# UDC-GAC/pRIblast

Hardware: AMD Instinct MI355X
Metric: query RNAs/sec in `ris` step (higher is better)
Workload: dtype f64

## Files before the change

priblast_amd/csrc/gapped_lds.hip:

```cpp
#include <algorithm>
#include <type_traits>

#include "gapped_args.hpp"
#include "search_device.hpp"
#include "search_kernels.hpp"

namespace prb {

#ifdef PRB_GAP_PROFILE
constexpr int kProfSlots = 31;
__device__ unsigned long long g_gap_prof[10 * kProfSlots];
struct GapProf {
  unsigned long long last, acc[kProfSlots];
  int cells_now = 0, cells_prev = 0;
  __device__ __forceinline__ void start() {
    for (int i = 0; i < kProfSlots; i++) acc[i] = 0;
    last = __builtin_amdgcn_s_memtime();
  }
  __device__ __forceinline__ void mark(int r) {
    const unsigned long long t = __builtin_amdgcn_s_memtime();
    if (t >= last) acc[r] += t - last;
    else acc[29] += 1;
    last = t;
  }
  __device__ __forceinline__ void count(int r) { acc[r] += 1; }
  __device__ __forceinline__ void flush(int kind) {
    if ((threadIdx.x & 63) == 0)
      for (int i = 0; i < kProfSlots; i++) atomicAdd(&g_gap_prof[kind * kProfSlots + i], acc[i]);
  }
};
#define GP_MARK(r) prof.mark(r)
#define GP_COUNT(r) prof.count(r)
#else
struct GapProf {
  __device__ __forceinline__ void start() {}
  __device__ __forceinline__ void flush(int) {}
};
#define GP_MARK(r)
#define GP_COUNT(r)
#endif

namespace {

constexpr int kInitStage = 16;
struct Tier0 {
#ifndef PRB_T0_CAPR
#define PRB_T0_CAPR 48
#define PRB_T0_WGCU 4
#endif
#ifndef PRB_T0_ACC_GLOBAL
#define PRB_T0_ACC_GLOBAL false
#endif
  static constexpr int kG = 8, kCapD = 32, kCapR = PRB_T0_CAPR, kGroups = 32, kWavesPerSimd = PRB_T0_WGCU, kWgPerCu = PRB_T0_WGCU;
  static constexpr bool kResumable = true;
  static constexpr bool kResumes = false;
  static constexpr bool kPairSteps = true;
  static constexpr bool kAccGlobal = PRB_T0_ACC_GLOBAL;
};
#ifndef PRB_T12_ACC_GLOBAL
#define PRB_T12_ACC_GLOBAL true
#endif
#ifndef PRB_T12_WPS
#define PRB_T12_WPS (PRB_T12_ACC_GLOBAL ? 4 : 3)
#endif
#ifndef PRB_T1_CAPD
#define PRB_T1_CAPD 40
#define PRB_T1_CAPR 64
#define PRB_T1_GROUPS 32
#define PRB_T1_WGCU (PRB_T12_ACC_GLOBAL ? 4 : 3)
#endif
struct Tier1 {
  static constexpr int kG = 8, kCapD = PRB_T1_CAPD, kCapR = PRB_T1_CAPR, kGroups = PRB_T1_GROUPS, kWavesPerSimd = PRB_T12_WPS, kWgPerCu = PRB_T1_WGCU;
  static constexpr bool kResumable = true, kResumes = true;
  using From = Tier0;
  using FromRec = Rec32;
  static constexpr bool kPairSteps = false;
  static constexpr bool kAccGlobal = PRB_T12_ACC_GLOBAL;
};
struct Tier2 {
  static constexpr int kG = 16, kCapD = 64, kCapR = 120, kGroups = 16, kWavesPerSimd = PRB_T12_WPS, kWgPerCu = PRB_T12_ACC_GLOBAL ? 4 : 3;
  static constexpr bool kResumable = true, kResumes = true;
  using From = Tier1;
  using FromRec = Rec32;
  static constexpr bool kPairSteps = false;
  static constexpr bool kAccGlobal = PRB_T12_ACC_GLOBAL;
};
struct Tier3 {
  static constexpr int kG = 64, kCapD = 128, kCapR = 512, kGroups = 1, kWavesPerSimd = 4, kWgPerCu = 16;
  static constexpr bool kResumable = false, kResumes = true;
  using From = Tier2;
  using FromRec = Rec32;
  static constexpr bool kPairSteps = false;
  static constexpr bool kAccGlobal = false;
};

struct Rec32W {
  using word = uint32_t;
  static constexpr bool kBases = false;
  static __device__ __forceinline__ word pack(int i, int j, int pred, int type, int, int) {
    return (word)i | ((word)j << 8) | ((word)pred << 16) | ((word)type << 25);
  }
  static __device__ __forceinline__ int i(word v) { return v & 0xFF; }
  static __device__ __forceinline__ int j(word v) { return (v >> 8) & 0xFF; }
  static __device__ __forceinline__ int pred(word v) { return (v >> 16) & 0x1FF; }
  static __device__ __forceinline__ int type(word v) { return (v >> 25) & 7; }
  static __device__ __forceinline__ int qa(word) { return 0; }
  static __device__ __forceinline__ int da(word) { return 0; }
};
struct Rec64 {
  using word = uint64_t;
  static constexpr bool kBases = true;
  static __device__ __forceinline__ word pack(int i, int j, int pred, int type, int qa, int da) {
    return (word)(uint32_t)i | ((word)(uint32_t)j << 16) | ((word)type << 32) | ((word)qa << 36) | ((word)da << 40) |
           ((word)(uint32_t)pred << 44);
  }
  static __device__ __forceinline__ int i(word v) { return (int)(v & 0xFFFF); }
  static __device__ __forceinline__ int j(word v) { return (int)((v >> 16) & 0xFFFF); }
  static __device__ __forceinline__ int pred(word v) { return (int)(v >> 44); }
  static __device__ __forceinline__ int type(word v) { return (int)((v >> 32) & 0xF); }
  static __device__ __forceinline__ int qa(word v) { return (int)((v >> 36) & 0xF); }
  static __device__ __forceinline__ int da(word v) { return (int)((v >> 40) & 0xF); }
};
static_assert(Tier3::kCapD + 16 <= 255 && Tier3::kCapR <= 512 && Tier0::kCapR * 8 >= 6 * kInitStage * 4 && Tier2::kCapD + 16 <= 127 && Tier2::kCapR <= 127, "Rec32 field widths");
static_assert(Tier0::kCapD <= Tier1::kCapD && Tier1::kCapD <= Tier2::kCapD && Tier2::kCapD <= Tier3::kCapD && Tier0::kCapR <= Tier1::kCapR &&
                  Tier1::kCapR <= Tier2::kCapR && Tier2::kCapR <= Tier3::kCapR,
              "a tier continues the dumps of the one before it");

template <class T, class Rec> struct LdsState {
  double eq[T::kCapD], ed[T::kCapD];
  double hyb[T::kCapR];
  typename Rec::word info[T::kCapR];
  static constexpr int kPtabLen = (T::kCapD + 7) & ~7;
  alignas(8) uint8_t ptab[3][kPtabLen];
  uint8_t qb[T::kCapD + 16], db[T::kCapD + 16];
};
template <class T, class Rec, bool kAccGlobal = T::kAccGlobal> struct LdsLive : LdsState<T, Rec> {};
template <class T, class Rec> struct LdsLive<T, Rec, true> {
  double hyb[T::kCapR];
  typename Rec::word info[T::kCapR];
  static constexpr int kPtabLen = (T::kCapD + 7) & ~7;
  alignas(8) uint8_t ptab[3][kPtabLen];
  uint8_t qb[T::kCapD + 16], db[T::kCapD + 16];
};
template <class T, class Rec> struct LdsStore {
  using R = Rec;
  static constexpr bool kResumable = T::kResumable;
  static constexpr bool kAccGlobal = T::kAccGlobal;
  static constexpr int kCapD = T::kCapD, kCapR = T::kCapR;
  LdsLive<T, Rec> &s;
  double *acc;
  __device__ __forceinline__ int cap_d() const { return T::kCapD; }
  __device__ __forceinline__ int cap_r() const { return T::kCapR; }
  __device__ __forceinline__ double &eq(int i) const {
    if constexpr (T::kAccGlobal) return acc[i];
    else return s.eq[i];
  }
  __device__ __forceinline__ double &ed(int i) const {
    if constexpr (T::kAccGlobal) return acc[T::kCapD + i];
    else return s.ed[i];
  }
  __device__ __forceinline__ double &hyb(int r) const { return s.hyb[r]; }
  __device__ __forceinline__ typename Rec::word &info(int r) const { return s.info[r]; }
  __device__ __forceinline__ uint8_t &ptab(int row, int i) const { return s.ptab[row][i]; }
  __device__ __forceinline__ int ptab_len() const { return LdsState<T, Rec>::kPtabLen; }
  __device__ __forceinline__ int win_len() const { return T::kCapD + 16; }
  __device__ __forceinline__ uint8_t &qb(int t) const { return s.qb[t]; }
  __device__ __forceinline__ uint8_t &db(int t) const { return s.db[t]; }
};
struct HbmStore {
  using R = Rec64;
  static constexpr bool kResumable = false;
  static constexpr bool kAccGlobal = false;
  double *eq_, *ed_, *hyb_;
  uint64_t *info_;
  uint8_t *ptab_, *qb_, *db_;
  int capd, capr;
  __device__ __forceinline__ int cap_d() const { return capd; }
  __device__ __forceinline__ int cap_r() const { return capr; }
  __device__ __forceinline__ double &eq(int i) const { return eq_[i]; }
  __device__ __forceinline__ double &ed(int i) const { return ed_[i]; }
  __device__ __forceinline__ double &hyb(int r) const { return hyb_[r]; }
  __device__ __forceinline__ uint64_t &info(int r) const { return info_[r]; }
  __device__ __forceinline__ uint8_t &ptab(int row, int i) const { return ptab_[(size_t)row * (capd + 4) + i]; }
  __device__ __forceinline__ int ptab_len() const { return capd + 4; }
  __device__ __forceinline__ int win_len() const { return capd + 16; }
  __device__ __forceinline__ uint8_t &qb(int t) const { return qb_[t]; }
  __device__ __forceinline__ uint8_t &db(int t) const { return db_[t]; }
};

template <bool kLds> __device__ __forceinline__ void group_sync() {
  if (kLds) {
    __builtin_amdgcn_fence(__ATOMIC_RELEASE, "wavefront");
    __builtin_amdgcn_wave_barrier();
    __builtin_amdgcn_fence(__ATOMIC_ACQUIRE, "wavefront");
  } else {
    __builtin_amdgcn_fence(__ATOMIC_RELEASE, "workgroup");
    __builtin_amdgcn_wave_barrier();
    __builtin_amdgcn_fence(__ATOMIC_ACQUIRE, "workgroup");
  }
}

template <class Store> __device__ __forceinline__ void acc_sync() {
  if constexpr (Store::kAccGlobal) {
    __builtin_amdgcn_fence(__ATOMIC_RELEASE, "workgroup");
    __builtin_amdgcn_wave_barrier();
    __builtin_amdgcn_fence(__ATOMIC_ACQUIRE, "workgroup");
  }
}

template <int kCtrl> __device__ __forceinline__ double dpp_f64(double x) {
  const int lo = __builtin_amdgcn_update_dpp(0, __double2loint(x), kCtrl, 0xF, 0xF, false);
  const int hi = __builtin_amdgcn_update_dpp(0, __double2hiint(x), kCtrl, 0xF, 0xF, false);
  return __hiloint2double(hi, lo);
}
template <int kCtrl> __device__ __forceinline__ int dpp_i32(int x) { return __builtin_amdgcn_update_dpp(0, x, kCtrl, 0xF, 0xF, false); }
__device__ __forceinline__ void group_min_halves(double &te, int &key, bool halves) {
  double m = te;
  m = __builtin_fmin(m, dpp_f64<0xB1>(m));
  m = __builtin_fmin(m, dpp_f64<0x4E>(m));
  const double m8 = __builtin_fmin(m, dpp_f64<0x141>(m));
  m = halves ? m : m8;
  int k = te == m ? key : 0x7fffffff;
  k = min(k, dpp_i32<0xB1>(k));
  k = min(k, dpp_i32<0x4E>(k));
  const int k8 = min(k, dpp_i32<0x141>(k));
  te = m;
  key = halves ? k : k8;
}
template <int G> __device__ __forceinline__ void group_min(double &te, int &key) {
// ... 451 lines not shown
          if (te < bte) {
            bte = te;
            bkp = (k << 3) | R::type(v);
          }
        }
      }
    }
    GP_MARK(4);
    group_min<16>(bte, bkp);
    GP_MARK(5);
    int bk = bkp >> 3, ptype = bkp & 7;
    if (d.lo >= dstart) bk = 0;
    if (ptype == 0) ptype = R::type(S.info(bk));
    if (act && sl == 0) {
      const int rec = d.nrec + sub;
      S.hyb(rec) = bte;
      S.info(rec) = R::pack(ci, cj, bk, rtype_of(ctype), fq, fd);
      S.ptab(cur, ci) = (uint8_t)ptype;
    }
    const double ie = eq_c + ed_c + bte;
#pragma unroll
    for (int t = 0; t < 4; t++) {
      if (t < n) {
        const int l16 = 16 * t;
        const double ie_t = __hiloint2double(__builtin_amdgcn_readlane(__double2hiint(ie), l16), __builtin_amdgcn_readlane(__double2loint(ie), l16));
        const int ci_t = __builtin_amdgcn_readlane(ci, l16);
        if (ie_t < d.min_e) {
          d.min_e = ie_t;
          d.best = d.nrec + t;
          d.min_ci = ci_t;
          d.min_cj = d.length - ci_t;
        }
      }
    }
    d.nrec += n;
    GP_MARK(6);
  };

  auto cell_type = [&](int i) -> int {
    if (i > i_hi) return 0;
    const int j = d.length - i;
    const unsigned q0 = S.qb(i), d0 = S.db(j), q1 = S.qb(i + 1), d1 = S.db(j + 1), q2 = S.qb(i + 2), d2b = S.db(j + 2);
    const int pt = S.ptab(d2, i - 1);
    const unsigned x0 = q0 * 5 + d0, x1 = q1 * 5 + d1, x2 = q2 * 5 + d2b;
    const unsigned p0 = (sc.pair_mask >> x0) & 1, w0 = (sc.wobble_mask >> x0) & 1;
    unsigned ahead = 1;
    if (min_helix >= 2) ahead = ((sc.pair_mask >> x1) & 1) & ~(w0 & (sc.wobble_mask >> x1));
    if (min_helix >= 3) ahead &= sc.pair_mask >> x2;
    for (int x = 3; x <= min_helix - 1; x++) ahead &= sc.pair_mask >> ((unsigned)S.qb(i + x) * 5 + S.db(j + x));
    const unsigned need = (unsigned)(pt == 0) | (w0 & (unsigned)wobble(pt));
    int t = (int)((sc.bp_rows >> ((x0 * 3 - 15) & 63)) & 7);
    if (flag == 1) t = ((t - 1) ^ 1) + 1;
    return (p0 & (ahead | ~need) & 1) ? t : 0;
  };

  if constexpr (G == 8 && kLds) {
    constexpr int kChunks = (Store::kCapD + G - 1) / G;
    using cells_t = typename std::conditional<kChunks <= 4, uint32_t, unsigned long long>::type;
    uint32_t tw[kChunks];
    cells_t cells = 0;
#pragma unroll
    for (int c = 0; c < kChunks; c++) {
      tw[c] = 0;
      const int i0 = i_lo + c * G;
      if (i0 <= i_hi) {
        const int type1 = cell_type(i0 + gl);
        uint32_t w = (uint32_t)type1 << (3 * gl);
        w |= (uint32_t)dpp_i32<0xB1>((int)w);
        w |= (uint32_t)dpp_i32<0x4E>((int)w);
        w |= (uint32_t)dpp_i32<0x141>((int)w);
        tw[c] = w;
        cells |= (cells_t)((__ballot(type1 != 0) >> gbase) & 0xFF) << (8 * c);
        GP_COUNT(11);
      }
    }
    GP_MARK(3);
#ifdef PRB_GAP_PROFILE
    prof.cells_now = kChunks <= 4 ? __popc((uint32_t)cells) : __popcll((unsigned long long)cells);
#endif
    while (cells) {
      const cells_t rest = cells & (cells - 1);
      const bool two = rest != 0 && d.nrec + 2 <= S.cap_r();
      const int b0 = kChunks <= 4 ? __builtin_ctz((uint32_t)cells) : __builtin_ctzll((unsigned long long)cells);
      if (Store::kResumable && d.nrec >= S.cap_r()) {
        d.overflow = true;
        d.resume_i0 = i_lo + b0;
        d.resume_dstart = dstart;
        break;
      }
      int b = b0;
      if (two) {
        const int b1 = kChunks <= 4 ? __builtin_ctz((uint32_t)rest) : __builtin_ctzll((unsigned long long)rest);
        if (gl >= G / 2) b = b1;
        cells = rest & (rest - 1);
      } else {
        cells = rest;
      }
      uint32_t w = tw[0];
#pragma unroll
      for (int c = 1; c < kChunks; c++) w = (b >> 3) == c ? tw[c] : w;
      const int ptype = fill_cell(i_lo + b, (int)((w >> (3 * (b & 7))) & 7), two);
      if (ptype < 0) {
        d.overflow = true;
        break;
      }
    }
    group_sync<kLds>();
    GP_MARK(3);
  } else {
    for (int i0 = i_lo; i0 <= i_hi && !d.overflow; i0 += G) {
      const int type1 = cell_type(i0 + gl);
      using mask_t = typename std::conditional<G <= 32, uint32_t, unsigned long long>::type;
      const unsigned long long tb0 = __ballot(type1 & 1), tb1 = __ballot(type1 & 2), tb2 = __ballot(type1 & 4);
      const unsigned long long anyb = tb0 | tb1 | tb2;
      mask_t vmask = G < 64 ? (mask_t)((anyb >> gbase) & ((1ull << (G & 63)) - 1)) : (mask_t)anyb;
      GP_MARK(3);
      GP_COUNT(11);
      if (Store::kResumable && d.nrec + __popcll((unsigned long long)vmask) > S.cap_r()) {
        d.overflow = true;
        d.resume_i0 = i0;
        d.resume_dstart = dstart;
        break;
      }
      while (vmask) {
        if constexpr (G == 64) {
          const int left = __popcll((unsigned long long)vmask), n = left < 4 ? left : 4;
          if (n >= 2 && d.nrec + n <= S.cap_r()) {
            fill_quad(i0, (unsigned long long)vmask, n, tb0, tb1, tb2);
            for (int t = 0; t < n; t++) vmask &= vmask - 1;
            continue;
          }
        }
        const int b = G <= 32 ? __builtin_ctz((uint32_t)vmask) : __builtin_ctzll((unsigned long long)vmask);
        vmask &= vmask - 1;
        const int ctype = (int)((tb0 >> (gbase + b)) & 1) | (int)(((tb1 >> (gbase + b)) & 1) << 1) |
                          (int)(((tb2 >> (gbase + b)) & 1) << 2);
        const int ptype = fill_cell(i0 + b, ctype, false);
        if (ptype < 0) {
          d.overflow = true;
          break;
        }
      }
      group_sync<kLds>();
      GP_MARK(3);
    }
  }
  if (d.overflow) return true;
  if (d.length - (d.min_ci + d.min_cj) >= drop) return true;
  if (!q_open && !d_open) return true;
  return false;
}


struct PairStep {
  uint32_t cellsA, cellsB;
  int LA, loA, loB, dstartA, i_loA, curA, typeA0, nrec;
  bool paired;
};

__device__ __forceinline__ int nth_bit(uint32_t m, int r) {
  int pos = 0;
#pragma unroll
  for (int w = 16; w >= 1; w >>= 1) {
    const int c = __popc(m & ((1u << w) - 1));
    if (r >= c) {
      r -= c;
      m >>= w;
      pos += w;
    }
  }
  return pos;
}

template <class Store> __device__ __forceinline__ int pair_type(const SearchConst &sc, const Store &S, int flag, int i, int j) {
  const unsigned x0 = (unsigned)S.qb(i) * 5 + S.db(j);
  int t = (int)((sc.bp_rows >> ((x0 * 3 - 15) & 63)) & 7);
  if (flag == 1) t = ((t - 1) ^ 1) + 1;
  return t;
}

template <class Store>
__device__ __forceinline__ bool pair_prep(const SearchConst &sc, const SeqBases &sb, const ExtOpts &o, const HitCtx &c, int flag,
                                          const Store &S, int gl, int gbase, DirState &d, PairStep &p, GapProf &prof) {
  constexpr int G = 8;
  using R = typename Store::R;
  static_assert(Store::kCapD <= 32, "a 32-bit mask of cells per anti-diagonal");
  constexpr int kChunks = (Store::kCapD + G - 1) / G;
  const int delta = o.delta, drop = o.drop_w_gap, min_helix = o.min_helix;
  const bool mid = d.resume_i0 != 0;
  if (!mid) {
    if (d.length >= S.cap_d()) {
      d.overflow = true;
      return true;
    }
    d.length++;
  }
  const int LA = d.length;
  const bool openA = LA < d.tq0 || LA < d.td0;
  const int curA = LA - 3 * ((LA * 171) >> 9), d2A = curA == 2 ? 0 : curA + 1;
  if (!mid) {
    if (LA > d.staged) stage_acc_regs<G, true>(sb, c, flag, delta, S, gl, gbase, d, LA);
    GP_MARK(1);
    GP_COUNT(10);
    uint64_t *row = reinterpret_cast<uint64_t *>(&S.ptab(curA, 0));
    for (int t = gl; t < S.ptab_len() / 8; t += G) row[t] = 0;
    group_sync<true>();
    if (LA - 2 > drop) {
      while (d.lo < d.nrec) {
        const auto v = S.info(d.lo);
        if (LA - R::i(v) - R::j(v) - 2 > drop) d.lo++;
        else break;
      }
    }
  }
  GP_MARK(2);
  const int dstartA = mid ? d.resume_dstart : d.nrec, loA = d.lo;
  const int i_firstA = LA - d.td0 + 1 > 1 ? LA - d.td0 + 1 : 1;
  const int i_loA = mid ? d.resume_i0 : i_firstA;
  const int i_hiA = (LA < d.tq0 ? LA : d.tq0) - 1;
  d.resume_i0 = 0;

  auto helix_ok = [&](unsigned x0, unsigned x1, unsigned x2, int pt, int i, int j) -> bool {
    const unsigned p0 = (sc.pair_mask >> x0) & 1, w0 = (sc.wobble_mask >> x0) & 1;
    unsigned ahead = 1;
    if (min_helix >= 2) ahead = ((sc.pair_mask >> x1) & 1) & ~(w0 & (sc.wobble_mask >> x1));
    if (min_helix >= 3) ahead &= sc.pair_mask >> x2;
    for (int x = 3; x <= min_helix - 1; x++) ahead &= sc.pair_mask >> ((unsigned)S.qb(i + x) * 5 + S.db(j + x));
    const unsigned need = (unsigned)(pt == 0) | (w0 & (unsigned)wobble(pt));
    return (p0 & (ahead | ~need) & 1) != 0;
  };

  const int LB = LA + 1, d2B = curA == 0 ? 2 : curA - 1;
  const bool try_pair = !mid && openA && LA - (d.min_ci + d.min_cj) < drop && LA < S.cap_d() && LB <= d.staged;
  uint32_t cellsA = 0, cellsB = 0;
  int loB = loA;
  bool paired = false;
  if (try_pair) {
    if (LB - 2 > drop) {
      while (loB < dstartA) {
        const auto v = S.info(loB);
        if (LB - R::i(v) - R::j(v) - 2 > drop) loB++;
        else break;
      }
    }
    const int i_loB = LB - d.td0 + 1 > 1 ? LB - d.td0 + 1 : 1, i_hiB = (LB < d.tq0 ? LB : d.tq0) - 1;
#pragma unroll
    for (int ch = 0; ch < kChunks; ch++) {
      const int i0 = i_loA + ch * G;
      if (i0 <= i_hiB) {
        const int i = i0 + gl, j = LA - i, jc = j < 0 ? 0 : j;
        const unsigned q0 = (unsigned)S.qb(i) * 5, q1 = (unsigned)S.qb(i + 1) * 5, q2 = (unsigned)S.qb(i + 2) * 5;
        const unsigned d0 = S.db(jc), d1 = S.db(jc + 1), d2b = S.db(jc + 2), d3 = S.db(jc + 3);
        const bool okA = i <= i_hiA && helix_ok(q0 + d0, q1 + d1, q2 + d2b, S.ptab(d2A, i - 1), i, j);
        const bool okB = i >= i_loB && i <= i_hiB && helix_ok(q0 + d1, q1 + d2b, q2 + d3, S.ptab(d2B, i - 1), i, j + 1);
        cellsA |= (uint32_t)((__ballot(okA) >> gbase) & 0xFF) << (8 * ch);
        cellsB |= (uint32_t)((__ballot(okB) >> gbase) & 0xFF) << (8 * ch);
        GP_COUNT(11);
      }
    }
    if (d.nrec + __popc(cellsA) + __popc(cellsB) <= S.cap_r()) {
      paired = true;
      uint64_t *row = reinterpret_cast<uint64_t *>(&S.ptab(d2A, 0));
      for (int t = gl; t < S.ptab_len() / 8; t += G) row[t] = 0;
      group_sync<true>();
      GP_COUNT(10);
    } else {
      cellsB = 0;
    }
  } else {
#pragma unroll
    for (int ch = 0; ch < kChunks; ch++) {
      const int i0 = i_loA + ch * G;
      if (i0 <= i_hiA) {
        const int i = i0 + gl, j = LA - i, jc = j < 0 ? 0 : j;
        const unsigned x0 = (unsigned)S.qb(i) * 5 + S.db(jc), x1 = (unsigned)S.qb(i + 1) * 5 + S.db(jc + 1),
                       x2 = (unsigned)S.qb(i + 2) * 5 + S.db(jc + 2);
        const bool okA = i <= i_hiA && helix_ok(x0, x1, x2, S.ptab(d2A, i - 1), i, j);
        cellsA |= (uint32_t)((__ballot(okA) >> gbase) & 0xFF) << (8 * ch);
        GP_COUNT(11);
      }
    }
  }
  const int nA = __popc(cellsA);
  int typeA0 = 0;
  if (paired && nA != 0) {
    const int iA0 = i_loA + __builtin_ctz(cellsA);
    typeA0 = rtype_of(pair_type(sc, S, flag, iA0, LA - iA0));
  }
#ifdef PRB_GAP_PROFILE
  prof.cells_now = nA + __popc(cellsB);
#endif
  const int room = S.cap_r() - d.nrec;
  if (nA > room) {
    const int keep = room > 0 ? room : 0, b = nth_bit(cellsA, keep);
    cellsA &= (1u << b) - 1;
    d.overflow = true;
    if (Store::kResumable) {
      d.resume_i0 = i_loA + b;
      d.resume_dstart = dstartA;
    }
  }
  p.cellsA = cellsA;
  p.cellsB = cellsB;
  p.LA = LA;
  p.loA = loA;
  p.loB = loB;
  p.dstartA = dstartA;
  p.i_loA = i_loA;
  p.curA = curA;
  p.typeA0 = typeA0;
  p.nrec = d.nrec;
  p.paired = paired;
  GP_MARK(3);
  return false;
}

template <class Store>
__device__ __forceinline__ void pair_cell(const SearchConst &sc, const Store &S, int flag, const PairStep &p, int b, int rec, int sub,
                                          int stride, bool halves, bool act, GapProf &prof) {
  using R = typename Store::R;
  GP_COUNT(12);
  const bool isB = b >= 32;
  const int cur = isB ? (p.curA == 2 ? 0 : p.curA + 1) : p.curA;
  const int lo = act ? (isB ? p.loB : p.loA) : 0, dstart = act ? p.dstartA : 0;
  const int ci = act ? p.i_loA + (b & 31) : 1, cj = act ? p.LA + (isB ? 1 : 0) - ci : 1;
  const int ctype = pair_type(sc, S, flag, ci, cj);
  const int nq = S.qb(ci - 1), nd = S.db(cj - 1);
  double bte = 1000000.0;
  int bkp = lo << 3;
  const typename R::word v0 = lo + sub < dstart ? S.info(lo + sub) : 0;
  scan_qualifying<R>(
      S, lo, dstart, sub, stride, ci, cj, v0,
      [&](typename R::word v) -> double {
        const int ri = R::i(v), rj = R::j(v);
        const int rq = R::qa(v), rd = R::da(v);
        const bool f0 = flag == 0;
        const int rt = R::type(v);
        return loop_energy_abcd(sc, f0 ? ctype : rt, f0 ? rt : ctype, ci - ri - 1, cj - rj - 1, f0 ? nq : rq, f0 ? nd : rd,
                                f0 ? rq : nq, f0 ? rd : nd);
      },
      bte, bkp, prof);
  GP_MARK(4);
  group_min_halves(bte, bkp, halves);
  GP_MARK(5);
  int bk = bkp >> 3, ptype = bkp & 7;
  const bool a_first = isB && p.typeA0 != 0 && lo >= dstart;
  if (lo >= dstart && !a_first) bk = 0;
  if (ptype == 0) ptype = a_first ? p.typeA0 : R::type(S.info(bk));
  if (act && sub == 0) {
    S.hyb(rec) = bte;
    S.info(rec) = R::pack(ci, cj, bk, rtype_of(ctype), S.qb(ci + 1), S.db(cj + 1));
    S.ptab(cur, ci) = (uint8_t)ptype;
  }
  GP_MARK(6);
}

template <class Store>
__device__ __forceinline__ void pair_fill_group(const SearchConst &sc, const Store &S, int flag, const PairStep &p, int gl, GapProf &prof) {
  unsigned long long cells = (unsigned long long)p.cellsA | ((unsigned long long)p.cellsB << 32);
  int rec = p.nrec;
  while (cells) {
    const unsigned long long rest = cells & (cells - 1);
    const bool two = rest != 0, hi = two && gl >= 4;
    const int b = hi ? __builtin_ctzll(rest) : __builtin_ctzll(cells);
    pair_cell(sc, S, flag, p, b, rec + (hi ? 1 : 0), two ? (gl & 3) : gl, two ? 4 : 8, two, true, prof);
    cells = two ? rest & (rest - 1) : rest;
    rec += two ? 2 : 1;
  }
  GP_MARK(26);
  group_sync<true>();
}

template <class T, class Rec>
__device__ __forceinline__ void pair_fill_pool(const SearchConst &sc, LdsLive<T, Rec> *wave_lds, int flag, const PairStep &p, int lane,
                                               GapProf &prof) {
  static_assert(T::kG == 8 && !T::kAccGlobal && T::kCapD < 255 && T::kCapR < 256, "eight groups per wavefront, state in LDS, 8-bit fields");
  const int n = __popc(p.cellsA) + __popc(p.cellsB);
  int incl[8];
  int total = 0;
#pragma unroll
  for (int g = 0; g < 8; g++) {
    total += __builtin_amdgcn_readlane(n, 8 * g);
    incl[g] = total;
  }
  group_sync<true>();
  const uint32_t pk0 = (uint32_t)p.LA | ((uint32_t)p.loA << 8) | ((uint32_t)p.loB << 16) | ((uint32_t)p.dstartA << 24);
  const uint32_t pk1 = (uint32_t)p.i_loA | ((uint32_t)p.curA << 8) | ((uint32_t)p.typeA0 << 10) | ((uint32_t)flag << 13) | ((uint32_t)p.nrec << 16);
  const int slot = lane >> 2, sub = lane & 3;
  for (int t0 = 0; t0 < total; t0 += 16) {
    GP_COUNT(30);
    const int t = t0 + slot;
    int o = 0, ex = 0;
#pragma unroll
    for (int g = 0; g < 7; g++) {
      if (t >= incl[g]) {
        o = g + 1;
        ex = incl[g];
      }
    }
    const int ob = 8 * o;
    const uint32_t q0 = __shfl(pk0, ob), q1 = __shfl(pk1, ob), cA = __shfl(p.cellsA, ob), cB = __shfl(p.cellsB, ob);
    PairStep po;
    po.cellsA = cA;
    po.cellsB = cB;
    po.LA = q0 & 0xFF;
    po.loA = (q0 >> 8) & 0xFF;
    po.loB = (q0 >> 16) & 0xFF;
    po.dstartA = q0 >> 24;
    po.i_loA = q1 & 0xFF;
    po.curA = (q1 >> 8) & 3;
    po.typeA0 = (q1 >> 10) & 7;
    po.nrec = q1 >> 16;
    po.paired = false;
    const int oflag = (q1 >> 13) & 1;
    const int rank = t - ex, nA = __popc(cA);
    const int b = rank < nA ? nth_bit(cA, rank) : 32 + nth_bit(cB, rank - nA);
    GP_MARK(28);
    const LdsStore<T, Rec> So{wave_lds[o], nullptr};
    pair_cell(sc, So, oflag, po, b, po.nrec + rank, sub, 4, true, t < total, prof);
  }
  group_sync<true>();
}

template <class Store>
__device__ __forceinline__ bool pair_close(const ExtOpts &o, const Store &S, int gl, DirState &d, const PairStep &p, GapProf &prof) {
  using R = typename Store::R;
  const int drop = o.drop_w_gap;
  const int n = __popc(p.cellsA) + __popc(p.cellsB);
  if (n != 0) {
    double m = __builtin_inf();
    int key = 0x7fffffff;
    for (int r = gl; r < n; r += 8) {
      const auto v = S.info(p.nrec + r);
      const double ie = S.eq(R::i(v) - 1) + S.ed(R::j(v) - 1) + S.hyb(p.nrec + r);
      if (ie < m) {
        m = ie;
        key = r;
      }
    }
    group_min<8>(m, key);
    if (m < d.min_e) {
      const auto v = S.info(p.nrec + key);
      d.min_e = m;
      d.best = p.nrec + key;
      d.min_ci = R::i(v);
      d.min_cj = R::j(v);
    }
    d.nrec = p.nrec + n;
  }
  GP_MARK(6);
  if (d.overflow) return true;
  if (p.paired) {
    d.length = p.LA + 1;
    d.lo = p.loB;
    if (p.LA + 1 - (d.min_ci + d.min_cj) >= drop) return true;
    return !(p.LA + 1 < d.tq0 || p.LA + 1 < d.td0);
  }
  if (p.LA - (d.min_ci + d.min_cj) >= drop) return true;
  return !(p.LA < d.tq0 || p.LA < d.td0);
}

template <class Store> __device__ __forceinline__ DirResult dir_finish(const DirState &d, HitState &h, int flag, const Store &S) {
  DirResult r;
  r.overflow = d.overflow;
  r.best = d.min_ci != 0 ? d.best : 0;
  if (d.min_ci != 0) {
    h.e_acc = h.e_acc + S.eq(d.min_ci - 1) + S.ed(d.min_cj - 1);
    if (flag == 0) {
      h.q_sp -= d.min_ci;
      h.db_sp -= d.min_cj;
    } else {
      h.id_start -= d.min_cj;
    }
    h.q_len += d.min_ci;
    h.db_len += d.min_cj;
  }
  h.e_tot = d.min_e;
  return r;
}

struct ResumeHeader {
  DirState d;
  double acc_prev1;
  HitState h;
  int32_t flag, nleft;
};
template <class T, class Rec> constexpr size_t resume_bytes() {
  return (sizeof(ResumeHeader) + sizeof(LdsState<T, Rec>) + 63) & ~(size_t)63;
}

template <int G, class T, class Rec>
__device__ __forceinline__ void resume_dump(const GapResume &ro, const HitCtx &c, const DirState &d, int flag,
                                            const LdsStore<T, Rec> &S, int gl, int gbase) {
  int slot = -1;
  if (gl == 0) {
    slot = (int)atomicAdd(ro.count, 1u);
    if (slot >= ro.cap) slot = -1;
  }
  slot = __shfl(slot, gbase);
  if (slot < 0) return;
  uint8_t *dst = ro.pool + (size_t)slot * resume_bytes<T, Rec>();
  ResumeHeader *H = reinterpret_cast<ResumeHeader *>(dst);
  if (gl == 0) {
    H->d = d;
    H->h = c.h;
    H->flag = flag;
    H->nleft = c.nleft;
    ro.slot[c.x] = slot;
  } else if (gl == 1) {
    H->acc_prev1 = d.acc_prev;
  }
  if constexpr (!T::kAccGlobal) {
    uint32_t *w = reinterpret_cast<uint32_t *>(dst + sizeof(ResumeHeader));
    const uint32_t *src = reinterpret_cast<const uint32_t *>(&S.s);
#pragma unroll 2
    for (int t = gl; t < (int)(sizeof(LdsState<T, Rec>) / 4); t += G) w[t] = src[t];
  } else {
    LdsState<T, Rec> *o = reinterpret_cast<LdsState<T, Rec> *>(dst + sizeof(ResumeHeader));
    for (int t = gl; t < T::kCapD; t += G) {
      o->eq[t] = S.eq(t);
      o->ed[t] = S.ed(t);
    }
    for (int t = gl; t < d.nrec; t += G) {
      o->hyb[t] = S.hyb(t);
      o->info[t] = S.info(t);
    }
    uint32_t *pw = reinterpret_cast<uint32_t *>(&o->ptab[0][0]);
    const uint32_t *ps = reinterpret_cast<const uint32_t *>(&S.s.ptab[0][0]);
    for (int t = gl; t < 3 * LdsState<T, Rec>::kPtabLen / 4; t += G) pw[t] = ps[t];
  }
}

template <int G, class TS, class RecS, class Store>
__device__ __forceinline__ void resume_load(const GapResume &ri, int slot, const GapArgs &a, HitCtx &c, DirState &d, int &flag,
                                            const Store &S, int gl) {
  using R = typename Store::R;
  const uint8_t *src = ri.pool + (size_t)slot * resume_bytes<TS, RecS>();
  const ResumeHeader *H = reinterpret_cast<const ResumeHeader *>(src);
  d = H->d;
  if (G > 1 && gl == 1) d.acc_prev = H->acc_prev1;
  d.overflow = false;
  c.h = H->h;
  c.nleft = H->nleft;
  flag = H->flag;
  const LdsState<TS, RecS> *s0 = reinterpret_cast<const LdsState<TS, RecS> *>(src + sizeof(ResumeHeader));
  stage_windows<G, true>(SeqBases{a.qb.enc, a.qb.acc, a.qb.cond, a.pg.acc, a.pg.cond}, c, flag, a.pg.seqs, a.pg.nchars, S, gl,
                         d);
  for (int t = gl; t < TS::kCapD; t += G) {
    S.eq(t) = s0->eq[t];
    S.ed(t) = s0->ed[t];
  }
  for (int t = gl; t < d.nrec; t += G) {
    S.hyb(t) = s0->hyb[t];
    const auto v = s0->info[t];
    S.info(t) = R::pack(RecS::i(v), RecS::j(v), RecS::pred(v), RecS::type(v), RecS::qa(v), RecS::da(v));
  }
  constexpr int kLenS = LdsState<TS, RecS>::kPtabLen;
  for (int t = gl; t < 3 * kLenS; t += G) {
    const int row = t / kLenS, i = t - row * kLenS;
    S.ptab(row, i) = s0->ptab[row][i];
  }
  group_sync<true>();
  acc_sync<Store>();
}

template <int kMode> __device__ __forceinline__ void hit_load(const GapArgs &a, int64_t w, HitCtx &c) {
  const SearchConst &sc = a.sc;
  const int64_t x = a.subset ? (int64_t)a.subset[w] : w;
  c.x = x;
  c.query = a.in.query[x];
  c.qo = a.qb.off[c.query];
  c.qn = a.qb.len[c.query] + 1;
  c.id = a.in.db_id[x];
  c.dbase = (int64_t)a.pg.start_pos[c.id] - c.id;
  HitState &h = c.h;
  h.q_sp = a.in.q_sp[x];
  h.db_sp = a.in.db_sp[x];
  h.q_len = a.in.q_len[x];
  h.db_len = a.in.db_len[x];
  h.id_start = a.in.db_id_start[x];
  h.e_tot = a.in.e_tot[x];
// ... 79 lines not shown
    a.overflow[w] = c.ovf ? 1 : 0;
    if (c.ovf && flag == 1) {
      const int64_t x = c.x;
      a.out.q_sp[x] = h.q_sp;
      a.out.db_sp[x] = h.db_sp;
      a.out.q_len[x] = h.q_len;
      a.out.db_len[x] = h.db_len;
      a.out.db_id_start[x] = h.id_start;
      a.out.e_acc[x] = h.e_acc;
      a.out.e_hyb[x] = h.e_tot - h.e_acc;
      a.out.e_tot[x] = h.e_tot;
      a.bp_count[x] = c.nleft;
      a.tier_out[x] = (uint8_t)(kResumeMark | ((c.resumed ? c.tier0 : a.tier_id) & kMarkTier));
    }
    if (!c.ovf) {
      const int64_t x = c.x;
      int tcode = a.tier_id > c.tier0 ? a.tier_id : c.tier0;
      if (a.tier_id == kWaveTier && a.lt.slot) {
        const int ls = a.lt.slot[x];
        if (ls >= 0) {
          const int c0 = a.lt.count[ls * 2], c1 = a.lt.count[ls * 2 + 1];
          if ((c0 >= 0 || (c0 == -1 && c.nleft <= kTraceCap)) && c1 >= 0) tcode = kLongTraceTier;
        }
      }
      a.tier_out[x] = (uint8_t)tcode;
      a.bp_count[x] = c.nleft | (c.nright << 16);
      const double d0 = dangle_energy_gapped(sc, h.q_sp, h.db_sp, 0, qs, c.qn, ds, a.pg.nchars);
      const double d1 = dangle_energy_gapped(sc, h.q_sp + US(h.q_len) - 1, (int64_t)h.db_sp + US(h.db_len) - 1, 1, qs, c.qn,
                                             ds, a.pg.nchars);
      double e = h.e_tot, hy = h.e_tot - h.e_acc;
      e += d0;
      e += d1;
      hy += d0;
      hy += d1;
      a.out.q_sp[x] = h.q_sp;
      a.out.db_sp[x] = h.db_sp;
      a.out.q_len[x] = h.q_len;
      a.out.db_len[x] = h.db_len;
      a.out.db_id[x] = c.id;
      a.out.db_id_start[x] = h.id_start;
      a.out.query[x] = c.query;
      a.out.e_acc[x] = h.e_acc;
      a.out.e_hyb[x] = hy;
      a.out.e_tot[x] = e;
    }
  } else if (!c.ovf) {
    int t = 0;
    const int64_t d0 = c.unsorted ? c.out0 : c.out0 + c.nleft;
    for (int u = 0; u < c.diag_len; u++)
      if (diag_pairs(sc, qs[c.diag_q + u], ds[c.diag_d + u])) {
        a.bp_out[2 * (d0 + t)] = c.diag_q + u;
        a.bp_out[2 * (d0 + t) + 1] = c.diag_d + u;
        t++;
      }
  }
}

__device__ __forceinline__ void hit_handover(const GapArgs &a, int64_t w, const HitCtx &c, int gl) {
  if (gl != 0) return;
  const int64_t x = c.x;
  const HitState &h = c.h;
  a.overflow[w] = 0;
  a.out.q_sp[x] = h.q_sp;
  a.out.db_sp[x] = h.db_sp;
  a.out.q_len[x] = h.q_len;
  a.out.db_len[x] = h.db_len;
  a.out.db_id_start[x] = h.id_start;
  a.out.e_acc[x] = h.e_acc;
  a.out.e_hyb[x] = h.e_tot - h.e_acc;
  a.out.e_tot[x] = h.e_tot;
  a.bp_count[x] = c.nleft;
  a.tier_out[x] = (uint8_t)(kHandoverMark | (a.tier_id & kMarkTier));
}

template <int kMode, class T, class Rec, bool kPair>
#ifdef PRB_TIERS_VGPR128
__global__ __launch_bounds__(T::kG *T::kGroups) __attribute__((amdgpu_num_vgpr(128))) void k_gapped_lds(GapArgs a) {
#else
__global__ __launch_bounds__(T::kG *T::kGroups, T::kWavesPerSimd) void k_gapped_lds(GapArgs a) {
#endif
  static_assert(!kPair || (T::kPairSteps && T::kG == 8), "pair steps");
  __shared__ LdsLive<T, Rec> lds[T::kGroups];
  constexpr int G = T::kG;
  const int gl = threadIdx.x & (G - 1);
  const int gbase = (threadIdx.x & 63) & ~(G - 1);
  const int gid = threadIdx.x / G;
  const LdsStore<T, Rec> S{lds[gid], T::kAccGlobal ? a.acc_scratch + ((size_t)blockIdx.x * T::kGroups + gid) * 2 * T::kCapD : nullptr};
  const int64_t ngroups = (int64_t)gridDim.x * T::kGroups;
  GapProf prof;
  prof.start();
  int64_t w = (int64_t)blockIdx.x * T::kGroups + gid;
  enum { kLoad, kInit, kRun, kFinished, kDone };
  int phase = w < a.n ? kLoad : kDone, flag = 0;
  const int period = a.period > 0 ? a.period : kPair ? (a.o.drop_w_gap > 1 ? (a.o.drop_w_gap + 1) / 2 : 1) : (a.o.drop_w_gap > 1 ? a.o.drop_w_gap : 1);
  int tick = 0;
  HitCtx c;
  DirState d;
  const SeqBases sb{a.qb.enc, a.qb.acc, a.qb.cond, a.pg.acc, a.pg.cond};
  while (__ballot(phase != kDone) != 0) {
    GP_MARK(14);
    if (a.early > 0 && tick != 0 && __popcll(__ballot(phase == kFinished)) >= a.early * G) tick = 0;
    if (tick == 0) {
      if (phase == kFinished) {
        DirResult r{true, 0};
        const DirOrigin og = dir_origin(c.h, flag);
        if (!d.overflow) {
          r = dir_finish(d, c.h, flag, S);
        } else {
          if constexpr (kMode == 0 && T::kResumable)
            if (a.rout.slot) resume_dump<G, T, Rec>(a.rout, c, d, flag, S, gl, gbase);
        }
        hit_dir_done<kMode, true>(a, c, flag, og, r, S, gl);
        group_sync<true>();
        GP_MARK(7);
        const bool hand = kMode == 0 && a.handover && !c.ovf && flag == 0 && !c.resumed;
        if (c.ovf || flag == 1 || hand) {
          if (hand) hit_handover(a, w, c, gl);
          else hit_store<kMode>(a, w, c, flag, gl);
          unsigned long long nw = 0;
          if (gl == 0) nw = (unsigned long long)ngroups + atomicAdd(a.next_work, 1ull);
          w = (int64_t)__shfl(nw, gbase);
          phase = w < a.n ? kLoad : kDone;
          GP_MARK(9);
        } else {
          flag = 1;
          phase = kInit;
        }
      }
      if (phase == kLoad) {
        hit_load<kMode>(a, w, c);
        flag = c.resumed ? 1 : 0;
        phase = kInit;
        if constexpr (kMode == 0 && T::kResumes) {
          const int slot = a.rin.slot ? a.rin.slot[c.x] : -1;
          if (slot >= 0) {
            resume_load<G, typename T::From, typename T::FromRec>(a.rin, slot, a, c, d, flag, S, gl);
            phase = kRun;
          }
        }
        GP_MARK(8);
      }
      if (phase == kInit) {
        dir_init<G, true>(a.sc, sb, c, flag, a.pg.seqs, a.pg.nchars, S, gl, a.o.delta, d);
        phase = kRun;
        GP_MARK(0);
      }
    }
    GP_MARK(15);
#ifdef PRB_GAP_PROFILE
    prof.cells_now = 0;
#endif
    if constexpr (kPair) {
      const bool run = phase == kRun;
      PairStep ps{0u, 0u, 0, 0, 0, 0, 0, 0, 0, 0, false};
      bool fin = false;
      if (run) fin = pair_prep(a.sc, sb, a.o, c, flag, S, gl, gbase, d, ps, prof);
      GP_MARK(run ? 3 : 27);
      if (a.pool) pair_fill_pool<T, Rec>(a.sc, &lds[gid & ~7], flag, ps, threadIdx.x & 63, prof);
      else if (run) pair_fill_group(a.sc, S, flag, ps, gl, prof);
      GP_MARK(run ? 26 : 27);
      if (run && (fin || pair_close(a.o, S, gl, d, ps, prof))) phase = kFinished;
      GP_MARK(run ? 6 : 27);
    } else {
      if (phase == kRun && dir_step<G, true>(a.sc, sb, a.o, c, flag, S, gl, gbase, d, prof)) phase = kFinished;
    }
#ifdef PRB_GAP_PROFILE
    if constexpr (G == 8) {
      auto wave_max = [](int v) {
        for (int m = 32; m >= 8; m >>= 1) {
          const int o = __shfl_xor(v, m);
          v = o > v ? o : v;
        }
        return v;
      };
      const int cn = prof.cells_now;
      prof.acc[16] += (unsigned long long)wave_max((cn + 1) / 2);
      prof.acc[17] += (unsigned long long)wave_max(cn);
      auto wave_sum = [](int v) {
        for (int m = 32; m >= 8; m >>= 1) v += __shfl_xor(v, m);
        return v;
      };
      prof.acc[18] += (unsigned long long)wave_sum(cn);
      if (tick & 1) {
        prof.acc[19] += (unsigned long long)wave_max((cn + prof.cells_prev + 1) / 2);
        prof.acc[20] += 1;
      } else {
        prof.cells_prev = cn;
      }
      prof.acc[21] += 1;
    }
#endif
    tick = tick + 1 == period ? 0 : tick + 1;
  }
  prof.flush(a.tier_id * 2 + (kMode != 0));
}

template <int kMode, bool kInLds> __global__ __launch_bounds__(64) void k_gapped_wave(GapArgs a, GapScratch scratch) {
  extern __shared__ __align__(16) uint8_t wave_smem[];
  const int gl = threadIdx.x;
  uint8_t *mine = kInLds ? wave_smem : scratch.base + (size_t)blockIdx.x * scratch.bytes_per_thread;
  HbmStore S;
  S.capd = scratch.cap_diag;
  S.capr = scratch.cap_rec;
  S.eq_ = reinterpret_cast<double *>(mine);
  S.ed_ = S.eq_ + S.capd;
  S.hyb_ = S.ed_ + S.capd;
  S.info_ = reinterpret_cast<uint64_t *>(S.hyb_ + S.capr);
  S.ptab_ = reinterpret_cast<uint8_t *>(S.info_ + S.capr);
  S.qb_ = S.ptab_ + 3 * ((size_t)S.capd + 4);
  S.db_ = S.qb_ + S.capd + 16;
  GapProf prof;
  prof.start();
  HitCtx c;
  DirState d;
  const SeqBases sb{a.qb.enc, a.qb.acc, a.qb.cond, a.pg.acc, a.pg.cond};
  for (int64_t w = blockIdx.x; w < a.n; w += gridDim.x) {
    hit_load<kMode>(a, w, c);
    int last = 0;
    bool hand = false;
    for (int flag = c.resumed ? 1 : 0; flag < 2 && !c.ovf && !hand; flag++) {
      GP_MARK(8);
      dir_init<64, false>(a.sc, sb, c, flag, a.pg.seqs, a.pg.nchars, S, gl, a.o.delta, d);
      GP_MARK(0);
      while (!dir_step<64, false>(a.sc, sb, a.o, c, flag, S, gl, 0, d, prof)) {
      }
      DirResult r{true, 0};
      const DirOrigin og = dir_origin(c.h, flag);
      if (!d.overflow) r = dir_finish(d, c.h, flag, S);
      hit_dir_done<kMode, false>(a, c, flag, og, r, S, gl);
      group_sync<false>();
      last = flag;
      hand = kMode == 0 && a.handover && !c.ovf && flag == 0 && !c.resumed;
      GP_MARK(7);
    }
    if (hand) hit_handover(a, w, c, gl);
    else hit_store<kMode>(a, w, c, last, gl);
    GP_MARK(9);
  }
  prof.flush(kWaveTier * 2 + (kMode != 0));
}

}

#ifdef PRB_GAP_PROFILE
extern "C" int prb_debug_gap_profile(unsigned long long *out, int reset) {
  if (hipDeviceSynchronize() != hipSuccess) return -1;
  if (hipMemcpyFromSymbol(out, HIP_SYMBOL(g_gap_prof), sizeof(unsigned long long) * 10 * kProfSlots) != hipSuccess) return -1;
  if (reset) {
    unsigned long long z[10 * kProfSlots] = {};
    if (hipMemcpyToSymbol(HIP_SYMBOL(g_gap_prof), z, sizeof(z)) != hipSuccess) return -1;
  }
  return 0;
}
#endif

size_t gapped_resume_bytes(int tier) {
  return tier == 0 ? resume_bytes<Tier0, Rec32>() : tier == 1 ? resume_bytes<Tier1, Rec32>() : resume_bytes<Tier2, Rec32>();
}

size_t gapped_acc_scratch_bytes() {
  if (!Tier1::kAccGlobal && !Tier0::kAccGlobal) return 0;
  const size_t t0 = (size_t)256 * Tier0::kWgPerCu * Tier0::kGroups * 2 * Tier0::kCapD * sizeof(double);
  const size_t t1 = (size_t)256 * Tier1::kWgPerCu * Tier1::kGroups * 2 * Tier1::kCapD * sizeof(double);
  const size_t t2 = (size_t)256 * Tier2::kWgPerCu * Tier2::kGroups * 2 * Tier2::kCapD * sizeof(double);
  return std::max(t0, std::max(t1, t2));
}

size_t gapped_wave_scratch_bytes(int cap_diag, int cap_rec) {
  size_t b = (size_t)cap_diag * 16 + (size_t)cap_rec * 16 + 3 * ((size_t)cap_diag + 4) + 2 * ((size_t)cap_diag + 16);
  return (b + 255) & ~(size_t)255;
}

namespace {
template <class T, class Rec> hipError_t launch_tier(GapArgs a, int mode, const GapTierKnobs &k, hipStream_t s) {
  const int64_t want = (a.n + T::kGroups - 1) / T::kGroups;
  const dim3 grid((unsigned)std::min<int64_t>(want, 256 * T::kWgPerCu)), blk(T::kG * T::kGroups);
  if (hipError_t e = hipMemsetAsync(a.next_work, 0, sizeof(unsigned long long), s); e != hipSuccess) return e;
  if constexpr (T::kPairSteps) {
    if (k.pair) {
      a.pool = k.pool;
      if (mode == 0) hipLaunchKernelGGL((k_gapped_lds<0, T, Rec, true>), grid, blk, 0, s, a);
      else hipLaunchKernelGGL((k_gapped_lds<2, T, Rec, true>), grid, blk, 0, s, a);
      return hipGetLastError();
    }
  }
  const size_t pad = k.pad_set ? (size_t)k.pad[a.tier_id < kLdsTiers ? a.tier_id : 0] : 0;
  if (mode == 0) hipLaunchKernelGGL((k_gapped_lds<0, T, Rec, false>), grid, blk, pad, s, a);
  else hipLaunchKernelGGL((k_gapped_lds<2, T, Rec, false>), grid, blk, 0, s, a);
  return hipGetLastError();
}
}

hipError_t launch_gapped_lds(const HitSoA &in, HitSoA out, int64_t n, const uint32_t *subset, const QBatchDev &qb,
                             const PageDev &pg, const SearchConst &sc, ExtOpts o, int mode, int tier, uint8_t *overflow,
                             uint8_t *tier_out, const uint8_t *first_flag, int32_t *bp_count, uint16_t *trace,
                             const int64_t *bp_off, int32_t *bp_out, unsigned long long *next_work, const GapResume &rin,
                             const GapResume &rout, const GapTierKnobs &knobs, hipStream_t s, int handover, double *acc_scratch) {
  if (n <= 0) return hipSuccess;
  GapArgs a{in,      out,   n,      subset, qb,        pg,         sc, o, overflow, tier_out, tier, first_flag, bp_count,
            trace,   bp_off, bp_out, next_work, rin,     rout};
  a.handover = mode == 0 ? handover : 0;
  a.acc_scratch = acc_scratch;
  if (((tier == 1 || tier == 2) && Tier1::kAccGlobal || tier == 0 && Tier0::kAccGlobal) && !acc_scratch) return hipErrorInvalidValue;
  const bool lds_tier = tier >= 0 && tier < kLdsTiers;
  if (knobs.period_set) a.period = mode == 0 && lds_tier ? knobs.period[tier] : 0;
  a.early = tier == 2 ? 2 : 0;
  if (knobs.early_set) a.early = lds_tier ? knobs.early[tier] : 0;
  if (tier == 0) return launch_tier<Tier0, Rec32>(a, mode, knobs, s);
  if (tier == 1) return launch_tier<Tier1, Rec32>(a, mode, knobs, s);
  if (tier == 2) return launch_tier<Tier2, Rec32>(a, mode, knobs, s);
  return launch_tier<Tier3, Rec32W>(a, mode, knobs, s);
}

hipError_t launch_gapped_wave(const HitSoA &in, HitSoA out, int64_t n, const uint32_t *subset, const QBatchDev &qb,
                              const PageDev &pg, const SearchConst &sc, ExtOpts o, GapScratch scratch, int mode,
                              uint8_t *overflow, uint8_t *tier_out, const uint8_t *first_flag, int32_t *bp_count,
                              const int64_t *bp_off, int32_t *bp_out, hipStream_t s, int handover, const LongTrace &lt) {
  if (n <= 0) return hipSuccess;
  GapArgs a{in,      out,    n,      subset,  qb,      pg,      sc,      o, overflow, tier_out, kWaveTier, first_flag, bp_count,
            nullptr, bp_off, bp_out, nullptr, GapResume{nullptr, nullptr, nullptr, 0}, GapResume{nullptr, nullptr, nullptr, 0}};
  a.handover = mode == 0 ? handover : 0;
  if (mode == 0) a.lt = lt;
  const int blocks = scratch.nthreads;
  if (scratch.base == nullptr) {
    const size_t lds = scratch.bytes_per_thread;
    if (mode == 0) hipLaunchKernelGGL((k_gapped_wave<0, true>), dim3(blocks), dim3(64), lds, s, a, scratch);
    else hipLaunchKernelGGL((k_gapped_wave<2, true>), dim3(blocks), dim3(64), lds, s, a, scratch);
  } else {
    if (mode == 0) hipLaunchKernelGGL((k_gapped_wave<0, false>), dim3(blocks), dim3(64), 0, s, a, scratch);
    else hipLaunchKernelGGL((k_gapped_wave<2, false>), dim3(blocks), dim3(64), 0, s, a, scratch);
  }
  return hipGetLastError();
}

}
```

Measured before the change: 7.721.

## Extend paired anti-diagonal steps to Tier1 with 64-bit cell masks

Enables the two-anti-diagonals-per-step path for Tier1 (capacity 40 diagonals), generalising the per-step cell masks from 32-bit to a templated 32/64-bit type with matching popcount, ctz and nth-bit helpers. For global-accumulator stores it stages accumulators one diagonal ahead so the paired B step has data, and passes the dynamic LDS pad to the paired launch. The aim is to halve per-diagonal group synchronisations and raise lane utilisation in Tier1 gapped extension, at the cost of wider masks, more register use and extra staging work.

```diff
diff --git a/priblast_amd/csrc/gapped_lds.hip b/priblast_amd/csrc/gapped_lds.hip
--- a/priblast_amd/csrc/gapped_lds.hip
+++ b/priblast_amd/csrc/gapped_lds.hip
@@ -8,7 +8,7 @@
 namespace prb {
 
 #ifdef PRB_GAP_PROFILE
-constexpr int kProfSlots = 31;
+constexpr int kProfSlots = 33;
 __device__ unsigned long long g_gap_prof[10 * kProfSlots];
 struct GapProf {
   unsigned long long last, acc[kProfSlots];
@@ -74,7 +74,7 @@
   static constexpr bool kResumable = true, kResumes = true;
   using From = Tier0;
   using FromRec = Rec32;
-  static constexpr bool kPairSteps = false;
+  static constexpr bool kPairSteps = true;
   static constexpr bool kAccGlobal = PRB_T12_ACC_GLOBAL;
 };
 struct Tier2 {
@@ -832,11 +832,18 @@
 }
 
 
-struct PairStep {
-  uint32_t cellsA, cellsB;
+template <int kCapD> using cell_mask_t = typename std::conditional<kCapD <= 32, uint32_t, uint64_t>::type;
+template <class M> struct PairStep {
+  using mask_t = M;
+  static constexpr int kBits = 8 * (int)sizeof(M);
+  M cellsA, cellsB;
   int LA, loA, loB, dstartA, i_loA, curA, typeA0, nrec;
   bool paired;
 };
+__device__ __forceinline__ auto mask_count(uint32_t m) { return __popc(m); }
+__device__ __forceinline__ int mask_count(uint64_t m) { return __popcll(m); }
+__device__ __forceinline__ int mask_first(uint32_t m) { return __builtin_ctz(m); }
+__device__ __forceinline__ int mask_first(uint64_t m) { return __builtin_ctzll(m); }
 
 __device__ __forceinline__ int nth_bit(uint32_t m, int r) {
   int pos = 0;
@@ -851,6 +858,19 @@
   }
   return pos;
 }
+__device__ __forceinline__ int nth_bit(uint64_t m, int r) {
+  int pos = 0;
+#pragma unroll
+  for (int w = 32; w >= 1; w >>= 1) {
+    const int c = __popcll(m & ((1ull << w) - 1));
+    if (r >= c) {
+      r -= c;
+      m >>= w;
+      pos += w;
+    }
+  }
+  return pos;
+}
 
 template <class Store> __device__ __forceinline__ int pair_type(const SearchConst &sc, const Store &S, int flag, int i, int j) {
   const unsigned x0 = (unsigned)S.qb(i) * 5 + S.db(j);
@@ -861,10 +881,12 @@
 
 template <class Store>
 __device__ __forceinline__ bool pair_prep(const SearchConst &sc, const SeqBases &sb, const ExtOpts &o, const HitCtx &c, int flag,
-                                          const Store &S, int gl, int gbase, DirState &d, PairStep &p, GapProf &prof) {
+                                          const Store &S, int gl, int gbase, DirState &d, PairStep<cell_mask_t<Store::kCapD>> &p,
+                                          GapProf &prof) {
   constexpr int G = 8;
   using R = typename Store::R;
-  static_assert(Store::kCapD <= 32, "a 32-bit mask of cells per anti-diagonal");
+  using M = cell_mask_t<Store::kCapD>;
+  static_assert(Store::kCapD <= 64, "a mask of cells per anti-diagonal");
   constexpr int kChunks = (Store::kCapD + G - 1) / G;
   const int delta = o.delta, drop = o.drop_w_gap, min_helix = o.min_helix;
   const bool mid = d.resume_i0 != 0;
@@ -879,7 +901,11 @@
   const bool openA = LA < d.tq0 || LA < d.td0;
   const int curA = LA - 3 * ((LA * 171) >> 9), d2A = curA == 2 ? 0 : curA + 1;
   if (!mid) {
-    if (LA > d.staged) stage_acc_regs<G, true>(sb, c, flag, delta, S, gl, gbase, d, LA);
+    if constexpr (Store::kAccGlobal) {
+      if (LA + 1 > d.staged && d.staged < S.cap_d()) stage_acc_regs<G, true>(sb, c, flag, delta, S, gl, gbase, d, d.staged + 1);
+    } else {
+      if (LA > d.staged) stage_acc_regs<G, true>(sb, c, flag, delta, S, gl, gbase, d, LA);
+    }
     GP_MARK(1);
     GP_COUNT(10);
     uint64_t *row = reinterpret_cast<uint64_t *>(&S.ptab(curA, 0));
@@ -912,7 +938,7 @@
 
   const int LB = LA + 1, d2B = curA == 0 ? 2 : curA - 1;
   const bool try_pair = !mid && openA && LA - (d.min_ci + d.min_cj) < drop && LA < S.cap_d() && LB <= d.staged;
-  uint32_t cellsA = 0, cellsB = 0;
+  M cellsA = 0, cellsB = 0;
   int loB = loA;
   bool paired = false;
   if (try_pair) {
@@ -933,12 +959,12 @@
         const unsigned d0 = S.db(jc), d1 = S.db(jc + 1), d2b = S.db(jc + 2), d3 = S.db(jc + 3);
         const bool okA = i <= i_hiA && helix_ok(q0 + d0, q1 + d1, q2 + d2b, S.ptab(d2A, i - 1), i, j);
         const bool okB = i >= i_loB && i <= i_hiB && helix_ok(q0 + d1, q1 + d2b, q2 + d3, S.ptab(d2B, i - 1), i, j + 1);
-        cellsA |= (uint32_t)((__ballot(okA) >> gbase) & 0xFF) << (8 * ch);
-        cellsB |= (uint32_t)((__ballot(okB) >> gbase) & 0xFF) << (8 * ch);
+        cellsA |= (M)((__ballot(okA) >> gbase) & 0xFF) << (8 * ch);
+        cellsB |= (M)((__ballot(okB) >> gbase) & 0xFF) << (8 * ch);
         GP_COUNT(11);
       }
     }
-    if (d.nrec + __popc(cellsA) + __popc(cellsB) <= S.cap_r()) {
+    if (d.nrec + mask_count(cellsA) + mask_count(cellsB) <= S.cap_r()) {
       paired = true;
       uint64_t *row = reinterpret_cast<uint64_t *>(&S.ptab(d2A, 0));
       for (int t = gl; t < S.ptab_len() / 8; t += G) row[t] = 0;
@@ -956,24 +982,24 @@
         const unsigned x0 = (unsigned)S.qb(i) * 5 + S.db(jc), x1 = (unsigned)S.qb(i + 1) * 5 + S.db(jc + 1),
                        x2 = (unsigned)S.qb(i + 2) * 5 + S.db(jc + 2);
         const bool okA = i <= i_hiA && helix_ok(x0, x1, x2, S.ptab(d2A, i - 1), i, j);
-        cellsA |= (uint32_t)((__ballot(okA) >> gbase) & 0xFF) << (8 * ch);
+        cellsA |= (M)((__ballot(okA) >> gbase) & 0xFF) << (8 * ch);
         GP_COUNT(11);
       }
     }
   }
-  const int nA = __popc(cellsA);
+  const int nA = mask_count(cellsA);
   int typeA0 = 0;
   if (paired && nA != 0) {
-    const int iA0 = i_loA + __builtin_ctz(cellsA);
+    const int iA0 = i_loA + mask_first(cellsA);
     typeA0 = rtype_of(pair_type(sc, S, flag, iA0, LA - iA0));
   }
 #ifdef PRB_GAP_PROFILE
-  prof.cells_now = nA + __popc(cellsB);
+  prof.cells_now = nA + mask_count(cellsB);
 #endif
   const int room = S.cap_r() - d.nrec;
   if (nA > room) {
     const int keep = room > 0 ? room : 0, b = nth_bit(cellsA, keep);
-    cellsA &= (1u << b) - 1;
+    cellsA &= ((M)1 << b) - 1;
     d.overflow = true;
     if (Store::kResumable) {
       d.resume_i0 = i_loA + b;
@@ -992,18 +1018,20 @@
   p.nrec = d.nrec;
   p.paired = paired;
   GP_MARK(3);
+  GP_COUNT(31);
+  if (paired) GP_COUNT(32);
   return false;
 }
 
-template <class Store>
-__device__ __forceinline__ void pair_cell(const SearchConst &sc, const Store &S, int flag, const PairStep &p, int b, int rec, int sub,
+template <class Store, class P>
+__device__ __forceinline__ void pair_cell(const SearchConst &sc, const Store &S, int flag, const P &p, int b, int rec, int sub,
                                           int stride, bool halves, bool act, GapProf &prof) {
   using R = typename Store::R;
   GP_COUNT(12);
-  const bool isB = b >= 32;
+  const bool isB = b >= P::kBits;
   const int cur = isB ? (p.curA == 2 ? 0 : p.curA + 1) : p.curA;
   const int lo = act ? (isB ? p.loB : p.loA) : 0, dstart = act ? p.dstartA : 0;
-  const int ci = act ? p.i_loA + (b & 31) : 1, cj = act ? p.LA + (isB ? 1 : 0) - ci : 1;
+  const int ci = act ? p.i_loA + (b & (P::kBits - 1)) : 1, cj = act ? p.LA + (isB ? 1 : 0) - ci : 1;
   const int ctype = pair_type(sc, S, flag, ci, cj);
   const int nq = S.qb(ci - 1), nd = S.db(cj - 1);
   double bte = 1000000.0;
@@ -1035,27 +1063,51 @@
   GP_MARK(6);
 }
 
-template <class Store>
-__device__ __forceinline__ void pair_fill_group(const SearchConst &sc, const Store &S, int flag, const PairStep &p, int gl, GapProf &prof) {
-  unsigned long long cells = (unsigned long long)p.cellsA | ((unsigned long long)p.cellsB << 32);
-  int rec = p.nrec;
-  while (cells) {
-    const unsigned long long rest = cells & (cells - 1);
-    const bool two = rest != 0, hi = two && gl >= 4;
-    const int b = hi ? __builtin_ctzll(rest) : __builtin_ctzll(cells);
-    pair_cell(sc, S, flag, p, b, rec + (hi ? 1 : 0), two ? (gl & 3) : gl, two ? 4 : 8, two, true, prof);
-    cells = two ? rest & (rest - 1) : rest;
-    rec += two ? 2 : 1;
+template <class Store, class P>
+__device__ __forceinline__ void pair_fill_group(const SearchConst &sc, const Store &S, int flag, const P &p, int gl, GapProf &prof) {
+  if constexpr (P::kBits == 32) {
+    unsigned long long cells = (unsigned long long)p.cellsA | ((unsigned long long)p.cellsB << 32);
+    int rec = p.nrec;
+    while (cells) {
+      const unsigned long long rest = cells & (cells - 1);
+      const bool two = rest != 0, hi = two && gl >= 4;
+      const int b = hi ? __builtin_ctzll(rest) : __builtin_ctzll(cells);
+      pair_cell(sc, S, flag, p, b, rec + (hi ? 1 : 0), two ? (gl & 3) : gl, two ? 4 : 8, two, true, prof);
+      cells = two ? rest & (rest - 1) : rest;
+      rec += two ? 2 : 1;
+    }
+  } else {
+    uint64_t ca = p.cellsA, cb = p.cellsB;
+    int rec = p.nrec;
+    auto take = [&]() -> int {
+      int b;
+      if (ca) {
+        b = __builtin_ctzll(ca);
+        ca &= ca - 1;
+      } else {
+        b = 64 + __builtin_ctzll(cb);
+        cb &= cb - 1;
+      }
+      return b;
+    };
+    while (ca | cb) {
+      const int b0 = take();
+      const bool two = (ca | cb) != 0, hi = two && gl >= 4;
+      const int b1 = two ? take() : b0;
+      pair_cell(sc, S, flag, p, hi ? b1 : b0, rec + (hi ? 1 : 0), two ? (gl & 3) : gl, two ? 4 : 8, two, true, prof);
+      rec += two ? 2 : 1;
+    }
   }
   GP_MARK(26);
   group_sync<true>();
 }
 
-template <class T, class Rec>
-__device__ __forceinline__ void pair_fill_pool(const SearchConst &sc, LdsLive<T, Rec> *wave_lds, int flag, const PairStep &p, int lane,
+template <class T, class Rec, class P>
+__device__ __forceinline__ void pair_fill_pool(const SearchConst &sc, LdsLive<T, Rec> *wave_lds, int flag, const P &p, int lane,
                                                GapProf &prof) {
-  static_assert(T::kG == 8 && !T::kAccGlobal && T::kCapD < 255 && T::kCapR < 256, "eight groups per wavefront, state in LDS, 8-bit fields");
-  const int n = __popc(p.cellsA) + __popc(p.cellsB);
+  using M = typename P::mask_t;
+  static_assert(T::kG == 8 && T::kCapD < 255 && T::kCapR < 256 && T::kCapD <= P::kBits, "eight groups per wavefront, 8-bit fields");
+  const int n = mask_count(p.cellsA) + mask_count(p.cellsB);
   int incl[8];
   int total = 0;
 #pragma unroll
@@ -1079,8 +1131,9 @@
       }
     }
     const int ob = 8 * o;
-    const uint32_t q0 = __shfl(pk0, ob), q1 = __shfl(pk1, ob), cA = __shfl(p.cellsA, ob), cB = __shfl(p.cellsB, ob);
-    PairStep po;
+    const uint32_t q0 = __shfl(pk0, ob), q1 = __shfl(pk1, ob);
+    const M cA = __shfl(p.cellsA, ob), cB = __shfl(p.cellsB, ob);
+    P po;
     po.cellsA = cA;
     po.cellsB = cB;
     po.LA = q0 & 0xFF;
@@ -1093,8 +1146,8 @@
     po.nrec = q1 >> 16;
     po.paired = false;
     const int oflag = (q1 >> 13) & 1;
-    const int rank = t - ex, nA = __popc(cA);
-    const int b = rank < nA ? nth_bit(cA, rank) : 32 + nth_bit(cB, rank - nA);
+    const int rank = t - ex, nA = mask_count(cA);
+    const int b = rank < nA ? nth_bit(cA, rank) : P::kBits + nth_bit(cB, rank - nA);
     GP_MARK(28);
     const LdsStore<T, Rec> So{wave_lds[o], nullptr};
     pair_cell(sc, So, oflag, po, b, po.nrec + rank, sub, 4, true, t < total, prof);
@@ -1102,11 +1155,11 @@
   group_sync<true>();
 }
 
-template <class Store>
-__device__ __forceinline__ bool pair_close(const ExtOpts &o, const Store &S, int gl, DirState &d, const PairStep &p, GapProf &prof) {
+template <class Store, class P>
+__device__ __forceinline__ bool pair_close(const ExtOpts &o, const Store &S, int gl, DirState &d, const P &p, GapProf &prof) {
   using R = typename Store::R;
   const int drop = o.drop_w_gap;
-  const int n = __popc(p.cellsA) + __popc(p.cellsB);
+  const int n = mask_count(p.cellsA) + mask_count(p.cellsB);
   if (n != 0) {
     double m = __builtin_inf();
     int key = 0x7fffffff;
@@ -1492,7 +1545,7 @@
 #endif
     if constexpr (kPair) {
       const bool run = phase == kRun;
-      PairStep ps{0u, 0u, 0, 0, 0, 0, 0, 0, 0, 0, false};
+      PairStep<cell_mask_t<T::kCapD>> ps{0u, 0u, 0, 0, 0, 0, 0, 0, 0, 0, false};
       bool fin = false;
       if (run) fin = pair_prep(a.sc, sb, a.o, c, flag, S, gl, gbase, d, ps, prof);
       GP_MARK(run ? 3 : 27);
@@ -1619,7 +1672,8 @@
   if constexpr (T::kPairSteps) {
     if (k.pair) {
       a.pool = k.pool;
-      if (mode == 0) hipLaunchKernelGGL((k_gapped_lds<0, T, Rec, true>), grid, blk, 0, s, a);
+      const size_t pad1 = k.pad_set && a.tier_id > 0 && a.tier_id < kLdsTiers ? (size_t)k.pad[a.tier_id] : 0;
+      if (mode == 0) hipLaunchKernelGGL((k_gapped_lds<0, T, Rec, true>), grid, blk, pad1, s, a);
       else hipLaunchKernelGGL((k_gapped_lds<2, T, Rec, true>), grid, blk, 0, s, a);
       return hipGetLastError();
     }
```

After: 7.629. -1.2%, worse.
